# sid2364/dna-sequences-pg-extension

Hardware: AMD Instinct MI355X
Metric: k-mers/sec for k=31 count over 3 Gbase synthetic; % of HBM-read roofline (higher is better)
Workload: dtype u64; 1 GPU; config 4: k=31 count over 3000000000 synthetic bases (splitmix64 seed 0xd2a0003), unordered groups (super-k-mer partitioning), single GPU; n_bases=3000000000, k=31, distinct=2999999968

## Files before the change

dna-sequences-pg-extension_amd/__init__.py:

```python
from .binding import (
    DEBUG_FORCE_SUPERKMER,
    DEBUG_GUARD_POOL,
    DEBUG_HEAVY_EXPAND,
    DEBUG_NO_SLAB0,
    DEBUG_NO_SPEC1,
    DEBUG_POISON_POOL,
    DEBUG_RANK_SMALL,
    DEBUG_SLAB0,
    DEBUG_SLAB0_OVERFLOW,
    DEBUG_SAMPLE1,
    DEBUG_SPEC1_OVERFLOW,
    Accumulator,
    Context,
    Dna,
    DnaGpuError,
    Filter,
    Hist,
    KmerIndex,
    Records,
    SPECTRUM_MAX_BINS,
    TOP_MAX,
    MULTI_AUTO,
    MULTI_COPY,
    MULTI_RCCL,
    Multi,
    ORDER_COUNT_ASC,
    ORDER_COUNT_DESC,
    Ranking,
    abi_version,
    device_count,
    kmer_count,
    lib,
# ... 4 lines not shown
```

dna-sequences-pg-extension_amd/binding.py:

```python
import ctypes as C
import os

import numpy as np

_HERE = os.path.dirname(os.path.abspath(__file__))
_LIB = None

OK = 0
ERR_INVALID_K = 1
ERR_QKMER_LEN_MISMATCH = 2
ERR_PREFIX_TOO_LONG = 3
ERR_QKMER_INVALID = 4
ERR_BAD_ARG = 5
ERR_TOO_LARGE = 6
ERR_NO_DEVICE = 7
ERR_OOM = 8
ERR_HIP = 9
ERR_DNA_EMPTY = 11
ERR_DNA_INVALID_CHAR = 12
DEBUG_POISON_POOL = 1
DEBUG_FORCE_SUPERKMER = 2
DEBUG_HEAVY_EXPAND = 4
DEBUG_GUARD_POOL = 8
DEBUG_NO_SPEC1 = 16
DEBUG_SPEC1_OVERFLOW = 32
DEBUG_SLAB0 = 64
DEBUG_NO_SLAB0 = 128
DEBUG_SLAB0_OVERFLOW = 256
DEBUG_SAMPLE1 = 512
DEBUG_RANK_SMALL = 1024
SPECTRUM_MAX_BINS = 1 << 20
TOP_MAX = 1 << 20
ORDER_COUNT_DESC = 0
ORDER_COUNT_ASC = 1
U64_MAX = 2 ** 64 - 1


def _env_debug():
    f = 0
    if os.environ.get("DNAGPU_TEST_POISON", "0") not in ("", "0"):
        f |= DEBUG_POISON_POOL
    if os.environ.get("DNAGPU_TEST_GUARD", "0") not in ("", "0"):
        f |= DEBUG_GUARD_POOL
    return f

FILTER_EQUALS = 1
FILTER_STARTS_WITH = 2
FILTER_CONTAINS = 3

MAX_PHASES = 48

u64p = C.POINTER(C.c_uint64)

# ... 973 lines not shown
```

dna-sequences-pg-extension_amd/csrc/kernels.hpp:

```cpp
#pragma once
#include <hip/hip_runtime.h>
#include <stdint.h>

#include "kmer_device.hpp"

namespace dnagpu {

hipError_t launch_synth(u64 *words, u64 w_begin, u64 w_end, u64 n_bases, u64 seed, u64 motif_len, hipStream_t s);
hipError_t launch_extract(const u64 *words, u64 n_words, u64 first, u64 count, int k, u64 *out_keys,
                          hipStream_t s);

constexpr int FILTER_MAX_GROUPS = 8192;
struct FilterSource {
    const u64 *words;
    u64 n_words;
    const u32 *marks;
    u64 n_mark_words;
    const u64 *seq_starts;
    u64 n_seqs;
};
void filter_bits_geometry(u64 count, u32 *n_groups, u32 *tiles_per_group);
hipError_t launch_filter_bits_count(const FilterSource &src, u64 first, u64 count, const FilterBits &fb, u32 *group_counts,
                                    hipStream_t s);
hipError_t launch_filter_bits_write(const FilterSource &src, u64 first, u64 count, const FilterBits &fb,
// ... 181 lines not shown
    const u32 *beg;
    u32 R;
    u32 C;
    int k;
    int test;
    FilterDev fd;
};
u32 index_scan_tiles(u64 C);
hipError_t launch_index_sweep_count(const IndexScanArgs &a, u32 *tile_counts, hipStream_t s);
hipError_t launch_index_sweep_write(const IndexScanArgs &a, const u32 *tile_offsets, u64 *out_rows, u64 *out_keys, u64 cap,
                                    hipStream_t s);
hipError_t launch_index_lookup(const u64 *r, u64 n, int k, const u64 *keys, u64 m, u64 *out_first, u64 *out_count, hipStream_t s);
hipError_t launch_index_read(const u64 *r, const u32 *row, int k, u64 first, u64 count, u64 *out_rows, u64 *out_keys, hipStream_t s);

int sk_min_k();
int sk_minimizer_len(int k);
int sk_tile_rows();
int sk_max_c0();
hipError_t launch_sk_level0(bool scatter, const Chunk *chunks, u32 n_chunks, const u64 *words, u64 n_words, u64 first, int k,
                            u32 c0n, u32 b1bits, u32 r0bits, u32 *hist, const u32 *tot, void *recs, hipStream_t s,
                            u32 *aux = nullptr, const u32 *marks = nullptr, u64 n_mark_words = 0);
hipError_t launch_sk_sample_chunks(Chunk *chunks, u32 n_chunks, u32 stride, u32 len, u32 n, hipStream_t s);
int sk_slab_words();
u32 sk_slab_cap(u32 est, u64 chunk_rows, u64 sampled);
hipError_t launch_sk_slab_init(const u32 *est, u32 r0bits, u32 chunk_rows, u32 sampled, u32 n_chunks, u32 *slab, Node *nodes,
                               hipStream_t s);
hipError_t launch_sk_hist1(const Node *nodes, const Chunk *chunks, u32 n_chunks, const void *recs, u32 *hist, u32 *kcount,
                           hipStream_t s, bool by_d2 = false);
hipError_t launch_sk_scatter1(const Node *nodes, const Chunk *chunks, u32 n_chunks, const void *src, void *dst, const u32 *hist,
                              const u32 *tot, hipStream_t s, bool by_d2 = false, u32 *gcur = nullptr);
u64 sk_spec_span(u32 len, int bits);
hipError_t launch_sk_spec_regions(const Node *nodes, u32 n_nodes, u32 *spec, u32 *out, u32 *gcur, hipStream_t s,
                                  const u32 *rstart = nullptr);
hipError_t launch_sk_scatter1_spec(const Node *nodes, const Chunk *chunks, u32 n_chunks, const void *src, void *dst, u32 *gcur,
                                   const u32 *spec, u32 *kcount, u32 *over, hipStream_t s, const u32 *rstart = nullptr,
                                   const u32 *rcap = nullptr);
hipError_t launch_sk_spec_nodes(const Node *nodes, u32 n_nodes, const u32 *spec, const u32 *gcur, Node *next, u32 *over,
                                hipStream_t s, const u32 *rstart = nullptr, const u32 *rcap = nullptr);
u32 sk_sample1_len();
u32 sk_sample1_every();
hipError_t launch_sk_sampled_regions(const Node *nodes, const Chunk *samples, u32 n_samples, const void *recs, u32 n_mid, u32 *est,
                                     u32 *rcap, u32 *rstart, u32 *scan_tmp, u32 *total, hipStream_t s);
hipError_t launch_sk_heavy_finals(const Node *kids, u32 n, const u32 *kcount, Node *out, hipStream_t s);
int sk_flat_slice();
hipError_t launch_sk_take_heavy(Node *mids, const u32 *idx, u32 n_heavy, const u32 *kcount, Node *out, hipStream_t s);
hipError_t launch_sk_slice_count(const Node *buckets, u32 nb, u32 *n_slices, hipStream_t s);
hipError_t launch_sk_slice_fill(const Node *buckets, u32 nb, const u32 *slice_first, u32 *slice_rec0, u32 *slice_nrec, hipStream_t s);
hipError_t launch_sk_slice_kmers(const void *recs, const u32 *slice_rec0, const u32 *slice_nrec, u32 n_slices, u32 *slice_km,
                                 hipStream_t s);
// ... 34 lines not shown
```

dna-sequences-pg-extension_amd/csrc/sk_host.hip:

```cpp
#include "host_common.hpp"

using namespace dnagpu;


constexpr u64 SK_LEAF_MEAN = 2500;
constexpr u64 SK_MID_LIMIT = (u64)1 << 27;
#ifndef SK_MID_RECORDS_LOG2
#define SK_MID_RECORDS_LOG2 16
#endif
constexpr u32 SK_MID_RECORDS = 1u << SK_MID_RECORDS_LOG2;
constexpr u64 SK_BIG_LIMIT = 0xFFFFFFFFull;
constexpr int SK_B1_MAX = 9;
constexpr u64 SK_SLAB_MIN_ROWS = (u64)1 << 29;

template <typename T>
static int alloc1(PoolScope &ps, size_t n, T **out, size_t per = 1)
{
    return ps.alloc(std::max<size_t>(n, 1) * per, out);
}

static u32 sk_chunk_len(u64 x, u64 target = 4096, u64 tile = 8192)
{
    const u64 len = std::max<u64>(4 * tile, (x + target - 1) / target);
    return (u32)((len + tile - 1) / tile * tile);
// ... 39 lines not shown
    RC_TRY(alloc1(ps, hc.n_chunks, &lv->chunks));
    RC_TRY(alloc1(ps, hc.n_chunks, &lv->hist, ROW_STRIDE));
    RC_TRY(alloc1(ps, hc.n_chunks, &lv->tot, ROW_STRIDE));
    RC_TRY(alloc1(ps, hc.n_next, &lv->next));
    HIP_TRY(launch_fill_chunks(cur, n_nodes, chunk_len, outc, nch, cur, lv->chunks, st));
    return DNAGPU_OK;
}

struct SkHeavy {
    Node *nodes = nullptr;
    u32 n = 0;
    bool counted = true;
    void *recs = nullptr;
    u64 total = 0;
};

struct SkParts {
    SkGeom g;
    int k = 0;
    u64 n_expected = 0;
    void *rec0 = nullptr;
    u64 rec0_cap = 0;
    u64 n_recs = 0;
    Node *coarse = nullptr;
    u32 n_coarse = 0;
    std::vector<u32> lens;
    void *recs = nullptr;
    Node *fin = nullptr;
    u32 n_fin = 0;
    SkHeavy heavy;
    u64 n_kmers = 0;
};

SkGeom dnagpu::sk_geometry(const dnagpu_ctx *ctx, u64 n, int k)
{
    SkGeom g;
    const u64 leaf_mean = std::min<u64>(SK_LEAF_MEAN, 225 * (u64)(k - sk_minimizer_len(k) + 2));
    const u64 n_final = std::max<u64>(n / leaf_mean, 16);
    const u64 n_mid = (n_final + 15) / 16;
    g.b1 = 1;
    while (g.b1 < SK_B1_MAX && ((u64)1 << g.b1) < n_mid)
        g.b1++;
    g.c0n = (u32)std::min<u64>((n_mid + ((u64)1 << g.b1) - 1) >> g.b1, (u64)sk_max_c0());
    g.r0bits = 1;
    while ((1u << g.r0bits) < g.c0n)
        g.r0bits++;
// ... 77 lines not shown
    RC_TRY(pool_alloc(ctx, (size_t)cap * 16, &rec0));
    ps.ptrs.push_back(rec0);
    prof_mark(ctx, "sk_scatter0");
    HIP_TRY(launch_sk_level0(true, l0.chunks, l0.n_chunks, dna->words, dna->n_words, rows.first, k, c0n, (u32)b1, (u32)r0bits,
                             l0.hist, l0.tot, rec0, st, nullptr, rows.marks, rows.n_mark_words));
    p.rec0 = rec0;
    p.rec0_cap = cap;
    p.coarse = l0.next;
    p.n_coarse = l0.n_next;
    p.n_recs = n_recs;
    return DNAGPU_OK;
}

static int sk_level0_slab(dnagpu_ctx *ctx, PoolScope &ps, SkParts &p, const SkRows &rows, bool *ok)
{
    hipStream_t st = ctx->stream;
    const dnagpu_dna *dna = rows.dna;
    const SkGeom &g = p.g;
    const int k = p.k;
    const u64 first = rows.first, n = rows.n;
    *ok = false;
    const u32 r0n = 1u << g.r0bits;
    const u64 tile = (u64)sk_tile_rows();
    Node *cur = nullptr;
    u32 chunk_rows = 0;
    SkLevel l0;
    RC_TRY(sk_level0_begin(ctx, ps, n, g.r0bits, 1024, &cur, &chunk_rows, &l0));
    if (l0.n_chunks == 0)
        return DNAGPU_OK;
    const u64 samp_len = 4 * tile, samp_stride = 64 * samp_len;
    const u32 n_samp = (u32)((n + samp_stride - 1) / samp_stride);
    u64 sampled = 0;
    for (u32 i = 0; i < n_samp; i++)
        sampled += std::min<u64>(samp_len, n - (u64)i * samp_stride);
    Chunk *samp = nullptr;
    u32 *est = nullptr, *slab = nullptr;
    Node *nodes = nullptr;
    RC_TRY(ps.alloc((size_t)n_samp, &samp));
    RC_TRY(ps.alloc((size_t)sk_max_c0(), &est));
    RC_TRY(ps.alloc((size_t)sk_slab_words(), &slab));
    RC_TRY(ps.alloc((size_t)r0n, &nodes));
    prof_mark(ctx, "sk_sample0");
    HIP_TRY(hipMemsetAsync(est, 0, (size_t)sk_max_c0() * sizeof(u32), st));
    HIP_TRY(launch_sk_sample_chunks(samp, n_samp, (u32)samp_stride, (u32)samp_len, (u32)n, st));
    HIP_TRY(launch_sk_level0(false, samp, n_samp, dna->words, dna->n_words, first, k, g.c0n, (u32)g.b1, (u32)g.r0bits, nullptr, nullptr,
                             nullptr, st, est, rows.marks, rows.n_mark_words));
    HIP_TRY(launch_sk_slab_init(est, (u32)g.r0bits, chunk_rows, (u32)sampled, l0.n_chunks, slab, nodes, st));
    std::vector<u32> h_est(r0n);
    RC_TRY(read_back(ctx, h_est.data(), est, (size_t)r0n * sizeof(u32)));
    u64 tot = 0, span = 0, span1 = 0;
    p.lens.assign(r0n, 0);
    for (u32 d = 0; d < r0n; d++) {
        tot += h_est[d];
        const u64 len = (u64)sk_slab_cap(h_est[d], chunk_rows, sampled) * l0.n_chunks;
        span += len;
        if (len > 0xFFFFFFFFull)
            return DNAGPU_OK;
        p.lens[d] = (u32)len;
        span1 += sk_spec_span((u32)len, g.b1);
    }
    if (tot == 0 || !sk_even(h_est.data(), r0n, 1.05) || span > 0xFFFFFFFFull)
        return DNAGPU_OK;
    const u64 cap = std::max<u64>(span, span1 <= 0xFFFFFFFFull ? span1 : 0);
    void *rec0 = nullptr;
    RC_TRY(pool_alloc(ctx, (size_t)std::max<u64>(cap, 1) * 16, &rec0));
    prof_mark(ctx, "sk_scatter0");
    const hipError_t e = launch_sk_level0(true, l0.chunks, l0.n_chunks, dna->words, dna->n_words, first, k, g.c0n, (u32)g.b1,
                                          (u32)g.r0bits, nullptr, nullptr, rec0, st, slab, rows.marks, rows.n_mark_words);
    u32 status[2] = {1, 0};
    int rc = e == hipSuccess ? read_back(ctx, status, slab + 18 * (size_t)sk_max_c0(), sizeof status) : DNAGPU_ERR_HIP;
    if (rc != DNAGPU_OK || status[0] || status[1] != (u32)span || (ctx->debug_flags & DNAGPU_DEBUG_SLAB0_OVERFLOW)) {
        pool_free(ctx, rec0);
        if (e != hipSuccess)
            set_err("sk_scatter0 (slabs): %s", hipGetErrorString(e));
        return rc;
    }
    ps.ptrs.push_back(rec0);
    p.rec0 = rec0;
    p.rec0_cap = cap;
    p.coarse = nodes;
    p.n_coarse = r0n;
    p.n_recs = span;
    *ok = true;
    return DNAGPU_OK;
}


struct SkL1 {
    SkLevel lv;
    u32 chunk_recs = 0;
    u32 *kcount = nullptr;
    u32 *d_lens = nullptr;
    u32 *gcur = nullptr;
    std::vector<u32> kc, rcn;
    u64 span = 0;
    u32 *rstart = nullptr, *rcapv = nullptr;
    void *rec1 = nullptr;
    bool rec1_kept = false;
};

enum class SkL1Route {
    Exact,
    Speculative,
    SpeculativeSampled,
};
// ... 76 lines not shown
    u32 total = 0;
    RC_TRY(read_back(ctx, &total, tot1, sizeof total));
    u64 chk = 0;
    for (u32 i = 0; i < n_coarse; i++)
        chk += host_lens[i];
    if ((u64)total >= chk && (u64)total <= p.rec0_cap) {
        l1.span = total;
        *route = SkL1Route::SpeculativeSampled;
    }
    return DNAGPU_OK;
}

static int sk_l1_speculative(dnagpu_ctx *ctx, PoolScope &ps, const SkParts &p, SkL1 &l1, SkL1Route route, bool *moved)
{
    hipStream_t st = ctx->stream;
    const bool sampled = route == SkL1Route::SpeculativeSampled;
    const u32 n_mid = l1.lv.n_next;
    u32 *const rstart = sampled ? l1.rstart : nullptr, *const rcapv = sampled ? l1.rcapv : nullptr;
    u32 *sp = nullptr;
    RC_TRY(ps.alloc((size_t)2 * p.n_coarse, &sp));
    u32 *status = l1.d_lens + n_mid;
    prof_mark(ctx, "sk_spec1");
    HIP_TRY(launch_sk_spec_regions(p.coarse, p.n_coarse, sp, status, l1.gcur, st, rstart));
    RC_TRY(pool_alloc(ctx, (size_t)std::max<u64>(std::max(p.n_recs, l1.span), 1) * 16, &l1.rec1));
    ps.ptrs.push_back(l1.rec1);
    prof_mark(ctx, "sk_scatter1");
    HIP_TRY(launch_sk_scatter1_spec(p.coarse, l1.lv.chunks, l1.lv.n_chunks, p.rec0, l1.rec1, l1.gcur, sp, l1.kcount, status + 2, st,
                                    rstart, rcapv));
    HIP_TRY(launch_sk_spec_nodes(p.coarse, p.n_coarse, sp, l1.gcur, l1.lv.next, status + 2, st, rstart, rcapv));
    HIP_TRY(launch_sk_node_lens(l1.lv.next, n_mid, l1.d_lens, st));
    RC_TRY(sk_l1_lens_to_host(ctx, l1, 3));
    const u32 *stw = l1.rcn.data() + n_mid;
    *moved = !((!sampled && stw[0] != (u32)l1.span) || (!sampled && stw[1]) || stw[2] ||
               (ctx->debug_flags & DNAGPU_DEBUG_SPEC1_OVERFLOW));
    if (!*moved)
        HIP_TRY(hipMemsetAsync(l1.kcount, 0, (size_t)std::max<u32>(n_mid, 1) * sizeof(u32), st));
    return DNAGPU_OK;
}

static int sk_l1_histogram(dnagpu_ctx *ctx, const SkParts &p, SkL1 &l1)
{
    hipStream_t st = ctx->stream;
    const SkLevel &lv = l1.lv;
    prof_mark(ctx, "sk_hist1");
    HIP_TRY(launch_sk_hist1(p.coarse, lv.chunks, lv.n_chunks, p.rec0, lv.hist, l1.kcount, st));
    prof_mark(ctx, "sk_prefix1");
    HIP_TRY(launch_level_prefix(p.coarse, lv.chunks, lv.n_chunks, p.n_coarse, l1.chunk_recs, lv.hist, lv.tot, st, p.n_coarse));
// ... 19 lines not shown
        set_err("super-k-mer partition lost rows: %llu of %llu", (unsigned long long)run, (unsigned long long)p.n_expected);
        return DNAGPU_ERR_INTERNAL;
    }
    if (run > 0xFFFFFFFFull)
        return DNAGPU_ERR_TOO_LARGE;
    p.n_kmers = run;
    if (!any_heavy)
        return DNAGPU_OK;
    for (u32 i = 0; i < n_mid; i++)
        if (is_heavy(i)) {
            heavy_idx->push_back(i);
            p.heavy.total += kc[i];
        }
    if (((debug_flags & DNAGPU_DEBUG_HEAVY_EXPAND) && p.heavy.total * 2 > run) || heavy_idx->size() > 32768)
        return DNAGPU_SK_SKEWED;
    return DNAGPU_OK;
}

static int sk_l1_scatter(dnagpu_ctx *ctx, PoolScope &ps, const SkParts &p, SkL1 &l1)
{
    hipStream_t st = ctx->stream;
    const SkLevel &lv = l1.lv;
    if (!l1.rec1) {
        RC_TRY(pool_alloc(ctx, (size_t)std::max<u64>(p.n_recs, 1) * 16, &l1.rec1));
        ps.ptrs.push_back(l1.rec1);
    }
    prof_mark(ctx, "sk_scatter1");
    HIP_TRY(hipMemcpyAsync(l1.gcur, lv.tot, (size_t)std::max<u32>(lv.n_chunks, 1) * ROW_STRIDE * sizeof(u32), hipMemcpyDeviceToDevice,
                           st));
    HIP_TRY(launch_sk_scatter1(p.coarse, lv.chunks, lv.n_chunks, p.rec0, l1.rec1, lv.hist, lv.tot, st, false, l1.gcur));
    return DNAGPU_OK;
}

struct SkSplit {
    SkLevel lv = {};
    u32 *kcount = nullptr;
};

static int sk_heavy_take(dnagpu_ctx *ctx, PoolScope &ps, SkParts &p, SkL1 &l1, const std::vector<u32> &heavy_idx, SkSplit *split)
{
    hipStream_t st = ctx->stream;
    const u32 nh = (u32)heavy_idx.size();
    u32 *d_idx = nullptr;
    Node *hnodes = nullptr;
    RC_TRY(ps.alloc((size_t)nh, &d_idx));
    RC_TRY(ps.alloc((size_t)nh, &hnodes));
    HIP_TRY(hipMemcpyAsync(d_idx, heavy_idx.data(), (size_t)nh * sizeof(u32), hipMemcpyHostToDevice, st));
// ... 507 lines not shown
```

dna-sequences-pg-extension_amd/csrc/superkmer_kernels.hip:

```cpp
#include <algorithm>
#include <cstdlib>
#include <type_traits>

#include "kernels.hpp"

namespace dnagpu {

constexpr int SK_NT = 256;
constexpr int SKW_ROWS = 63 * 32;
constexpr int SK_TILE_ROWS = (SK_NT / 64) * SKW_ROWS;
constexpr int SK_MAX_C0 = 256;
constexpr int SKW_LIST = 768;
__host__ __device__ constexpr u32 sk_plain_max(int w) { return (u32)(2 * SKW_ROWS * 17 / (10 * (w + 1))) < (u32)SKW_LIST ? (u32)(2 * SKW_ROWS * 17 / (10 * (w + 1))) : (u32)SKW_LIST; }

int sk_tile_rows() { return SK_TILE_ROWS; }
int sk_max_c0() { return SK_MAX_C0; }
int sk_count_cap() { return 4096; }

typedef unsigned long long ull2_t __attribute__((ext_vector_type(2)));

constexpr int SK_REC_MULTI_BIT = 58;
constexpr int SK_POS_SHIFT = 39;
constexpr u32 SK_POS_MASK = 31u;
constexpr u32 SK_GPOS_MASK = 63u;

__device__ __forceinline__ u32 sk_mix_raw(u32 t, u32 hi_bits )
{
    return __umul24(t, 0x9E3779u) + __umul24(__builtin_amdgcn_ubfe(t, 24u, hi_bits), 0x85EBCBu);
}
__device__ __forceinline__ u32 sk_mix(u32 v) { return sk_mix_raw(v, 8u); }

struct SkDigits {
    u32 d0, d1, d2;
};
__device__ __forceinline__ u32 sk_digit_word(u32 hmin) { return __umul24(hmin >> 7, 0x9E3779u); }
__device__ __forceinline__ u32 sk_digit0(u32 g, u32 c0) { return __umul24(g >> 16, c0) >> 16; }
__device__ __forceinline__ u32 sk_fine_word(u32 v) { return v * 0x9E3779B1u; }
__device__ __forceinline__ SkDigits sk_digits(u32 hmin, u32 v, u32 c0, u32 b1mask)
{
// ... 345 lines not shown
                    atomicAdd(&h[sk_digit0(sk_digit_word(fm.hm[0]), c0n)], ((u32)SKW_ROWS + lmax - 1u) / lmax);
            } else {
                sk_hist0_general<W, BATCH>(fm, words, n_words, first + ch.off + t0, lmax, mmask, c0n, h);
            }
        }
    }
    __syncthreads();
    if (accum) {
        for (u32 d = threadIdx.x; d < r0n; d += SK_NT)
            if (h[d])
                atomicAdd(&accum[d], h[d]);
        return;
    }
    u32 *row = hist + (u64)blockIdx.x * ROW_STRIDE;
    for (u32 d = threadIdx.x; d < r0n; d += SK_NT)
        row[d] = h[d];
}

struct SkBuild {
    u64 *wl;
    const u64 *wsh;
    u32 *gpos;
    const u32 *gend;
    ull2_t *recs;
    u32 fo, c0n, b1mask, mmask;
    int k, dbg;
};

template <bool BATCH>
__device__ __forceinline__ bool sk_build(const SkBuild &b, u32 wrun, int mode)
{
    const bool exact = mode != 0;
    const int dbg = b.dbg;
    (void)dbg;
    bool dropped = false;
    if (SK_DBG(2))
        return false;
    for (u32 e = threadIdx.x & 63u; e < wrun; e += 64) {
        const u64 en = b.wl[e];
        const u32 key = (u32)(en >> 32);
        if (BATCH && (exact ? key < 64u : key == ~0u))
            continue;
        const u32 end_row = (u32)en & 0xFFFFu;
        u32 v = key, hmin = key;
        if (exact) {
            const u32 xq = (end_row & ~31u) + (key & SK_GPOS_MASK) + b.fo;
// ... 9 lines not shown
        const u32 len = end_row - start + 1u;
        const u32 q = start + b.fo;
        const u32 wi = q >> 5, sh = (q & 15u) * 2u;
        const u64 a0 = b.wsh[wi], a1 = b.wsh[wi + 1], a2 = b.wsh[wi + 2];
        const bool odd = (q & 16u) != 0;
        const u32 e0 = odd ? (u32)(a0 >> 32) : (u32)a0, e1 = odd ? (u32)a1 : (u32)(a0 >> 32),
                  e2 = odd ? (u32)(a1 >> 32) : (u32)a1, e3 = odd ? (u32)a2 : (u32)(a1 >> 32),
                  e4 = odd ? (u32)(a2 >> 32) : (u32)a2;
        u64 lo = ((u64)__builtin_amdgcn_alignbit(e2, e1, sh) << 32) | __builtin_amdgcn_alignbit(e1, e0, sh);
        u64 hi = ((u64)__builtin_amdgcn_alignbit(e4, e3, sh) << 32) | __builtin_amdgcn_alignbit(e3, e2, sh);
        const u32 nb = len + (u32)b.k - 1;
        if (nb < 32) {
            lo &= ((u64)1 << (2 * nb)) - 1;
            hi = 0;
        } else {
            hi &= ((u64)1 << (2 * (nb - 32))) - 1;
        }
        const u32 mpos = (end_row & ~31u) + (key & SK_GPOS_MASK) - start;
        const u32 tag = exact ? (mpos & SK_POS_MASK) << (SK_POS_SHIFT - 32) : 1u << (SK_REC_MULTI_BIT - 32);
        hi |= ((u64)(len - 1) << 44) | ((u64)dg.d1 << 49) | ((u64)dg.d2 << 59) | ((u64)tag << 32);
        ull2_t r;
        r.x = lo;
        r.y = hi;
        if (gslot >= b.gend[dg.d0])
            dropped = true;
        else if (!SK_DBG(1))
            b.recs[gslot] = r;
        else if (r.x == 0x1234567 && r.y == 0x89)
            b.recs[0] = r;
    }
    return dropped;
}

template <int W, bool BATCH, bool BYV>
__device__ __forceinline__ bool sk_scatter0_walk(SkFront<W> &f, const SkBuild &bx, const u64 *__restrict__ words, u64 n_words,
                                                 u64 tile_pos, u32 lmax)
{
    const u64 below = ((u64)1 << (threadIdx.x & 63)) - 1;
    u64 *wl = bx.wl;
    bool dropped = false;
    SkKeys<W, BATCH, BYV> key(f, words, n_words, tile_pos, bx.mmask);
    sk_front_open<W>(f, key, lmax);
    for (int n_pass = BYV ? 1 : 4, pass = 0; pass < n_pass; pass++) {
        const int jlo = pass * (32 / n_pass), jhi = jlo + 32 / n_pass;
        u32 wrun = 0;
        key.forget();
        sk_records_all<W>(f, key, lmax, [&](int j, bool end_any, u32 end_row, u32 len, u32, u32 kj) {
            const bool end = end_any && j >= jlo && j < jhi;
            const u64 b = __ballot(end);
// ... 45 lines not shown
        for (u32 d = tid; d < r0n; d += SK_NT) {
            const u32 cap = slab[d];
            const u32 base = cap ? atomicAdd(&slab[SK_MAX_C0 + 16 * d], cap) : 0u;
            gpos[d] = base;
            gbeg[d] = base;
            gend[d] = base + cap;
        }
    } else {
        const u32 *hrow = hist + (u64)blockIdx.x * ROW_STRIDE;
        const u32 *trow = tot;
        for (u32 d = tid; d < r0n; d += SK_NT) {
            gpos[d] = trow[d] + hrow[d];
            gend[d] = ~0u;
        }
    }
    __syncthreads();
    u64 *wsh = wsh_all[wave], *wl = list_all[wave];
    bool dropped = false;
    SkBuild bx;
    bx.wl = wl;
    bx.wsh = wsh;
    bx.gpos = gpos;
    bx.gend = gend;
    bx.recs = recs;
    bx.fo = 0;
    bx.c0n = c0n;
    bx.b1mask = b1mask;
    bx.mmask = mmask;
    bx.k = k;
    bx.dbg = dbg;
    for (u32 t0 = (u32)wave * SKW_ROWS; t0 < ch.len; t0 += SK_TILE_ROWS) {
        const u32 n_rows = ch.len - t0 < (u32)SKW_ROWS ? ch.len - t0 : (u32)SKW_ROWS;
        const u64 tile_pos = first + ch.off + t0;
        const u32 fo = (u32)(tile_pos & 31);
        SkFront<W> f;
        sk_front<W, BATCH>(f, words, n_words, tile_pos, n_rows, lmax, mmask, wsh, marks, n_mark_words);
        bx.fo = fo;
        auto build = [&](u32 wrun, int mode) {
            if (sk_build<BATCH>(bx, wrun, mode))
                dropped = true;
        };
        if (f.plain) {
            const u32 nf = lane == 62 ? ~f.hm[31] : f.next_first;
            u32 cnt = 0;
#pragma unroll
            for (int j = 0; j < 32; j++)
// ... 19 lines not shown
            }
        }
        {
            SkFront<W> fm = f;
            const SkBuild bm = bx;
            const u32 uv = fm.plain ? sk_uniform_value<W, BATCH>(fm, words, n_words, tile_pos, mmask) : ~0u;
            if (uv != ~0u) {
                const u32 n_rec = ((u32)SKW_ROWS + lmax - 1u) / lmax;
                for (u32 e = (u32)lane; e < n_rec; e += 64) {
                    const u32 s0 = e * lmax, e1 = (s0 + lmax < (u32)SKW_ROWS ? s0 + lmax : (u32)SKW_ROWS) - 1u;
                    wl[e] = ((u64)uv << 32) | (u64)((s0 << 16) | e1);
                }
                sk_wave_fence();
                if (sk_build<BATCH>(bm, n_rec, 0))
                    dropped = true;
                sk_wave_fence();
            } else if (sk_scatter0_general<W, BATCH>(fm, bm, words, n_words, tile_pos, lmax)) {
                dropped = true;
            }
        }
    }
    if (slab) {
        if (dropped)
            slab[18 * SK_MAX_C0] = 1u;
        __syncthreads();
        ull2_t null_rec;
        null_rec.x = 0;
        null_rec.y = (unsigned long long)1 << 63;
        for (u32 d = (u32)wave; d < r0n; d += SK_NT / 64) {
            const u32 e = gend[d], u = gpos[d] < e ? gpos[d] : e;
            for (u32 i = u + (u32)lane; i < e; i += 64)
                __builtin_nontemporal_store(null_rec, &recs[i]);
            if (lane == 0 && u > gbeg[d])
                atomicAdd(&slab[17 * SK_MAX_C0 + d], u - gbeg[d]);
        }
    }
}

__global__ __launch_bounds__(256) void sk_sample_chunks_kernel(Chunk *__restrict__ chunks, u32 n_chunks, u32 stride, u32 len, u32 n)
{
    const u32 i = blockIdx.x * blockDim.x + threadIdx.x;
    if (i >= n_chunks)
        return;
    const u64 off = (u64)i * stride;
    Chunk c;
    c.node = 0;
    c.off = (u32)off;
    c.len = off >= (u64)n ? 0u : (u32)((u64)len < (u64)n - off ? (u64)len : (u64)n - off);
    c.pad = 0;
    chunks[i] = c;
}

__host__ __device__ inline u32 sk_isqrt(u64 v)
{
    u64 r = 0, bit = (u64)1 << 62;
    while (bit > v)
        bit >>= 2;
    while (bit) {
        if (v >= r + bit) {
            v -= r + bit;
            r = (r >> 1) + bit;
        } else {
            r >>= 1;
        }
        bit >>= 2;
    }
    return (u32)r;
}
__host__ __device__ inline u32 sk_slab_cap_of(u32 est, u64 chunk_rows, u64 sampled)
{
    if (est == 0)
        return 0;
    const u64 e = ((u64)est * chunk_rows) / sampled + 1;
    return (u32)((e + e / 32 + 6 * (u64)sk_isqrt(e) + 24 + 7) & ~(u64)7);
}
u32 sk_slab_cap(u32 est, u64 chunk_rows, u64 sampled) { return sk_slab_cap_of(est, chunk_rows, sampled); }

__global__ __launch_bounds__(SK_MAX_C0) void sk_slab_init_kernel(const u32 *__restrict__ est, u32 r0n, u32 chunk_rows, u32 sampled,
                                                                u32 n_chunks, u32 child_meta, u32 *__restrict__ slab,
                                                                Node *__restrict__ nodes)
{
    __shared__ u64 sc[SK_MAX_C0];
    const u32 d = threadIdx.x;
    const u32 cap = d < r0n ? sk_slab_cap_of(est[d], chunk_rows, sampled) : 0u;
    sc[d] = (u64)cap * n_chunks;
    __syncthreads();
    if (d == 0) {
        u64 run = 0;
        for (u32 i = 0; i < (u32)SK_MAX_C0; i++) {
            const u64 c = sc[i];
            sc[i] = run;
            run += c;
        }
        slab[18 * SK_MAX_C0] = 0;
        slab[18 * SK_MAX_C0 + 1] = (u32)(run < 0xFFFFFFFFull ? run : 0xFFFFFFFFull);
    }
    __syncthreads();
    if (d < r0n) {
        const u32 start = (u32)(sc[d] < 0xFFFFFFFFull ? sc[d] : 0xFFFFFFFFull);
        slab[d] = cap;
        slab[SK_MAX_C0 + 16 * d] = start;
        slab[17 * SK_MAX_C0 + d] = 0;
        Node o;
        o.start = start;
        o.len = cap * n_chunks;
        o.meta = child_meta;
        o.split = 0;
        o.prefix = 0;
        o.child_base = 0;
        o.chunk_base = 0;
        nodes[d] = o;
    }
}

constexpr int SK1_NT = 1024;
__global__ __launch_bounds__(SK1_NT) void sk_hist1_kernel(const Node *__restrict__ nodes, const Chunk *__restrict__ chunks,
                                                          u32 n_chunks, const ull2_t *__restrict__ recs,
                                                          u32 *__restrict__ hist, u32 *__restrict__ kcount, int shift)
{
    __shared__ u32 h[ROW_STRIDE];
    __shared__ u32 kc[ROW_STRIDE];
    if (blockIdx.x >= n_chunks)
        return;
    const Chunk ch = chunks[blockIdx.x];
    const Node nd = nodes[ch.node];
    const u32 R = 1u << nd.split;
    for (u32 d = threadIdx.x; d < R; d += SK1_NT) {
        h[d] = 0;
        kc[d] = 0;
    }
    __syncthreads();
    const u64 *hi = reinterpret_cast<const u64 *>(recs + (u64)nd.start + ch.off) + 1;
    u32 i = threadIdx.x;
    for (; i + 3u * SK1_NT < ch.len; i += 4u * SK1_NT) {
        u64 m[4];
// ... 1918 lines not shown
    const u32 b1mask = (1u << b1bits) - 1, r0n = 1u << r0bits;
    if (r0n > (u32)SK_MAX_C0)
        return hipErrorInvalidValue;
#define SK_CASE(W_) case W_: \
        if (marks) launch_front<W_, true>(scatter, n_chunks, s, chunks, words, n_words, first, k, lmax, mmask, c0n, b1mask, r0n, hist, tot, recs, aux, marks, n_mark_words); \
        else launch_front<W_, false>(scatter, n_chunks, s, chunks, words, n_words, first, k, lmax, mmask, c0n, b1mask, r0n, hist, tot, recs, aux, nullptr, 0); \
        break;
    switch (w) {
        SK_CASE(9) SK_CASE(10) SK_CASE(11) SK_CASE(12) SK_CASE(13) SK_CASE(14) SK_CASE(15) SK_CASE(16) SK_CASE(17) SK_CASE(18)
    default: return hipErrorInvalidValue;
    }
#undef SK_CASE
    return hipGetLastError();
}

hipError_t launch_sk_sample_chunks(Chunk *chunks, u32 n_chunks, u32 stride, u32 len, u32 n, hipStream_t s)
{
    if (n_chunks == 0)
        return hipSuccess;
    hipLaunchKernelGGL(sk_sample_chunks_kernel, dim3((n_chunks + 255) / 256), dim3(256), 0, s, chunks, n_chunks, stride, len, n);
    return hipGetLastError();
}

int sk_slab_words() { return 18 * SK_MAX_C0 + 4; }

hipError_t launch_sk_slab_init(const u32 *est, u32 r0bits, u32 chunk_rows, u32 sampled, u32 n_chunks, u32 *slab, Node *nodes,
                               hipStream_t s)
{
    hipLaunchKernelGGL(sk_slab_init_kernel, dim3(1), dim3(SK_MAX_C0), 0, s, est, 1u << r0bits, chunk_rows, sampled, n_chunks,
                       (u32)(32 - r0bits), slab, nodes);
    return hipGetLastError();
}

hipError_t launch_sk_hist1(const Node *nodes, const Chunk *chunks, u32 n_chunks, const void *recs, u32 *hist, u32 *kcount,
                           hipStream_t s, bool by_d2)
{
    if (n_chunks == 0)
        return hipSuccess;
    hipLaunchKernelGGL(sk_hist1_kernel, dim3(n_chunks), dim3(SK1_NT), 0, s, nodes, chunks, n_chunks,
                       reinterpret_cast<const ull2_t *>(recs), hist, kcount, by_d2 ? 59 : 49);
    return hipGetLastError();
}

hipError_t launch_sk_scatter1(const Node *nodes, const Chunk *chunks, u32 n_chunks, const void *src, void *dst, const u32 *hist,
                              const u32 *tot, hipStream_t s, bool by_d2, u32 *gcur)
{
    if (n_chunks == 0)
        return hipSuccess;
    hipLaunchKernelGGL(sk_scatter1_kernel<false>, dim3(n_chunks), dim3(SK1_NT), 0, s, nodes, chunks, n_chunks,
                       reinterpret_cast<const ull2_t *>(src), reinterpret_cast<ull2_t *>(dst), hist, tot, by_d2 ? 59 : 49, gcur,
                       nullptr, nullptr, nullptr, nullptr, nullptr);
    return hipGetLastError();
}
// ... 75 lines not shown
```

include/dnagpu.h:

```cpp
#ifndef DNAGPU_H
#define DNAGPU_H

#include <stdint.h>
#include <stddef.h>

#ifdef __cplusplus
extern "C" {
#endif

#define DNAGPU_ABI_VERSION 2

#define DNAGPU_OK                       0
#define DNAGPU_ERR_INVALID_K            1
#define DNAGPU_ERR_QKMER_LEN_MISMATCH   2
#define DNAGPU_ERR_PREFIX_TOO_LONG      3
#define DNAGPU_ERR_QKMER_INVALID        4
#define DNAGPU_ERR_BAD_ARG              5
#define DNAGPU_ERR_TOO_LARGE            6
#define DNAGPU_ERR_NO_DEVICE            7
#define DNAGPU_ERR_OOM                  8
#define DNAGPU_ERR_HIP                  9
#define DNAGPU_ERR_INTERNAL             10
#define DNAGPU_ERR_DNA_EMPTY            11
#define DNAGPU_ERR_DNA_INVALID_CHAR     12
// ... 202 lines not shown
int dnagpu_kmer_index_build(dnagpu_ctx *ctx, const uint64_t *keys, uint64_t n, int k, int on_device, dnagpu_kmer_index **out);
uint64_t dnagpu_kmer_index_rows(const dnagpu_kmer_index *idx);
uint64_t dnagpu_kmer_index_distinct(const dnagpu_kmer_index *idx);
int dnagpu_kmer_index_k(const dnagpu_kmer_index *idx);
int dnagpu_kmer_index_scan(dnagpu_ctx *ctx, const dnagpu_kmer_index *idx, const dnagpu_filter *filter, uint64_t *out_rows,
                           uint64_t *out_keys, uint64_t cap, uint64_t *n_out, uint64_t *visited, int out_on_device);
int dnagpu_kmer_index_lookup(dnagpu_ctx *ctx, const dnagpu_kmer_index *idx, const uint64_t *keys, uint64_t m,
                             uint64_t *out_first, uint64_t *out_count, int on_device);
int dnagpu_kmer_index_read(dnagpu_ctx *ctx, const dnagpu_kmer_index *idx, uint64_t first, uint64_t count, uint64_t *out_rows,
                           uint64_t *out_keys, int out_on_device);
void dnagpu_kmer_index_free(dnagpu_ctx *ctx, dnagpu_kmer_index *idx);

#define DNAGPU_DEBUG_POISON_POOL 1u
#define DNAGPU_DEBUG_FORCE_SUPERKMER 2u
#define DNAGPU_DEBUG_HEAVY_EXPAND 4u
#define DNAGPU_DEBUG_GUARD_POOL 8u
#define DNAGPU_DEBUG_NO_SPEC1 16u
#define DNAGPU_DEBUG_SPEC1_OVERFLOW 32u
#define DNAGPU_DEBUG_SLAB0 64u
#define DNAGPU_DEBUG_NO_SLAB0 128u
#define DNAGPU_DEBUG_SLAB0_OVERFLOW 256u
#define DNAGPU_DEBUG_SAMPLE1 512u
#define DNAGPU_DEBUG_RANK_SMALL 1024u
int dnagpu_set_debug(dnagpu_ctx *ctx, unsigned flags);

#define DNAGPU_MAX_PHASES 48
typedef struct dnagpu_phase_times {
    int         n;
    const char *names[DNAGPU_MAX_PHASES];
    float       ms[DNAGPU_MAX_PHASES];
} dnagpu_phase_times;
int dnagpu_last_phase_times(dnagpu_ctx *ctx, dnagpu_phase_times *out);
int dnagpu_multi_last_phase_times(dnagpu_multi *m, int rank, dnagpu_phase_times *out);
int dnagpu_set_profiling(dnagpu_ctx *ctx, int enabled);

#ifdef __cplusplus
}
#endif
#endif
```

Measured before the change: 164.7 billion k-mers/s.

## Add per-bucket overflow areas to level-0 slab scatter and shrink slab padding

New measurement: 167.1 billion k-mers/s (median of 3 runs). About the same (+1.5%).

```diff
diff --git a/dna-sequences-pg-extension_amd/__init__.py b/dna-sequences-pg-extension_amd/__init__.py
--- a/dna-sequences-pg-extension_amd/__init__.py
+++ b/dna-sequences-pg-extension_amd/__init__.py
@@ -7,7 +7,9 @@
     DEBUG_POISON_POOL,
     DEBUG_RANK_SMALL,
     DEBUG_SLAB0,
+    DEBUG_SLAB0_NO_AREA,
     DEBUG_SLAB0_OVERFLOW,
+    DEBUG_SLAB0_TIGHT,
     DEBUG_SAMPLE1,
     DEBUG_SPEC1_OVERFLOW,
     Accumulator,
diff --git a/dna-sequences-pg-extension_amd/binding.py b/dna-sequences-pg-extension_amd/binding.py
--- a/dna-sequences-pg-extension_amd/binding.py
+++ b/dna-sequences-pg-extension_amd/binding.py
@@ -29,6 +29,8 @@
 DEBUG_SLAB0_OVERFLOW = 256
 DEBUG_SAMPLE1 = 512
 DEBUG_RANK_SMALL = 1024
+DEBUG_SLAB0_TIGHT = 2048
+DEBUG_SLAB0_NO_AREA = 4096
 SPECTRUM_MAX_BINS = 1 << 20
 TOP_MAX = 1 << 20
 ORDER_COUNT_DESC = 0
diff --git a/dna-sequences-pg-extension_amd/csrc/kernels.hpp b/dna-sequences-pg-extension_amd/csrc/kernels.hpp
--- a/dna-sequences-pg-extension_amd/csrc/kernels.hpp
+++ b/dna-sequences-pg-extension_amd/csrc/kernels.hpp
@@ -227,9 +227,12 @@
                             u32 *aux = nullptr, const u32 *marks = nullptr, u64 n_mark_words = 0);
 hipError_t launch_sk_sample_chunks(Chunk *chunks, u32 n_chunks, u32 stride, u32 len, u32 n, hipStream_t s);
 int sk_slab_words();
-u32 sk_slab_cap(u32 est, u64 chunk_rows, u64 sampled);
-hipError_t launch_sk_slab_init(const u32 *est, u32 r0bits, u32 chunk_rows, u32 sampled, u32 n_chunks, u32 *slab, Node *nodes,
-                               hipStream_t s);
+constexpr u32 SK_SLAB_TIGHT = 1, SK_SLAB_NO_AREA = 2;
+u32 sk_slab_cap(u32 est, u64 chunk_rows, u64 sampled, u32 mode);
+u64 sk_slab_area(u32 est, u64 chunk_rows, u64 sampled, u32 n_chunks, u32 mode);
+hipError_t launch_sk_slab_init(const u32 *est, u32 r0bits, u32 chunk_rows, u32 sampled, u32 n_chunks, u32 mode, u32 *slab,
+                               Node *nodes, hipStream_t s);
+hipError_t launch_sk_slab_close(u32 r0bits, u32 *slab, Node *nodes, hipStream_t s);
 hipError_t launch_sk_hist1(const Node *nodes, const Chunk *chunks, u32 n_chunks, const void *recs, u32 *hist, u32 *kcount,
                            hipStream_t s, bool by_d2 = false);
 hipError_t launch_sk_scatter1(const Node *nodes, const Chunk *chunks, u32 n_chunks, const void *src, void *dst, const u32 *hist,
diff --git a/dna-sequences-pg-extension_amd/csrc/sk_host.hip b/dna-sequences-pg-extension_amd/csrc/sk_host.hip
--- a/dna-sequences-pg-extension_amd/csrc/sk_host.hip
+++ b/dna-sequences-pg-extension_amd/csrc/sk_host.hip
@@ -85,6 +85,7 @@
     void *rec0 = nullptr;
     u64 rec0_cap = 0;
     u64 n_recs = 0;
+    u64 rec0_span = 0;
     Node *coarse = nullptr;
     u32 n_coarse = 0;
     std::vector<u32> lens;
@@ -208,6 +209,8 @@
     *ok = false;
     const u32 r0n = 1u << g.r0bits;
     const u64 tile = (u64)sk_tile_rows();
+    const u32 mode = ((ctx->debug_flags & DNAGPU_DEBUG_SLAB0_TIGHT) ? SK_SLAB_TIGHT : 0u) |
+                     ((ctx->debug_flags & DNAGPU_DEBUG_SLAB0_NO_AREA) ? SK_SLAB_NO_AREA : 0u);
     Node *cur = nullptr;
     u32 chunk_rows = 0;
     SkLevel l0;
@@ -231,18 +234,18 @@
     HIP_TRY(launch_sk_sample_chunks(samp, n_samp, (u32)samp_stride, (u32)samp_len, (u32)n, st));
     HIP_TRY(launch_sk_level0(false, samp, n_samp, dna->words, dna->n_words, first, k, g.c0n, (u32)g.b1, (u32)g.r0bits, nullptr, nullptr,
                              nullptr, st, est, rows.marks, rows.n_mark_words));
-    HIP_TRY(launch_sk_slab_init(est, (u32)g.r0bits, chunk_rows, (u32)sampled, l0.n_chunks, slab, nodes, st));
+    HIP_TRY(launch_sk_slab_init(est, (u32)g.r0bits, chunk_rows, (u32)sampled, l0.n_chunks, mode, slab, nodes, st));
     std::vector<u32> h_est(r0n);
     RC_TRY(read_back(ctx, h_est.data(), est, (size_t)r0n * sizeof(u32)));
-    u64 tot = 0, span = 0, span1 = 0;
-    p.lens.assign(r0n, 0);
+    u64 tot = 0, span = 0, span1 = 0, slab_slots = 0;
     for (u32 d = 0; d < r0n; d++) {
         tot += h_est[d];
-        const u64 len = (u64)sk_slab_cap(h_est[d], chunk_rows, sampled) * l0.n_chunks;
+        const u64 slabs = (u64)sk_slab_cap(h_est[d], chunk_rows, sampled, mode) * l0.n_chunks;
+        const u64 len = slabs + sk_slab_area(h_est[d], chunk_rows, sampled, l0.n_chunks, mode);
+        slab_slots += slabs;
         span += len;
         if (len > 0xFFFFFFFFull)
             return DNAGPU_OK;
-        p.lens[d] = (u32)len;
         span1 += sk_spec_span((u32)len, g.b1);
     }
     if (tot == 0 || !sk_even(h_est.data(), r0n, 1.05) || span > 0xFFFFFFFFull)
@@ -251,22 +254,41 @@
     void *rec0 = nullptr;
     RC_TRY(pool_alloc(ctx, (size_t)std::max<u64>(cap, 1) * 16, &rec0));
     prof_mark(ctx, "sk_scatter0");
-    const hipError_t e = launch_sk_level0(true, l0.chunks, l0.n_chunks, dna->words, dna->n_words, first, k, g.c0n, (u32)g.b1,
-                                          (u32)g.r0bits, nullptr, nullptr, rec0, st, slab, rows.marks, rows.n_mark_words);
-    u32 status[2] = {1, 0};
-    int rc = e == hipSuccess ? read_back(ctx, status, slab + 18 * (size_t)sk_max_c0(), sizeof status) : DNAGPU_ERR_HIP;
+    hipError_t e = launch_sk_level0(true, l0.chunks, l0.n_chunks, dna->words, dna->n_words, first, k, g.c0n, (u32)g.b1,
+                                    (u32)g.r0bits, nullptr, nullptr, rec0, st, slab, rows.marks, rows.n_mark_words);
+    if (e == hipSuccess)
+        e = launch_sk_slab_close((u32)g.r0bits, slab, nodes, st);
+    std::vector<u32> status(4 + (size_t)r0n, 0);
+    status[0] = 1;
+    int rc = e == hipSuccess ? read_back(ctx, status.data(), slab + 18 * (size_t)sk_max_c0(), status.size() * sizeof(u32))
+                             : DNAGPU_ERR_HIP;
     if (rc != DNAGPU_OK || status[0] || status[1] != (u32)span || (ctx->debug_flags & DNAGPU_DEBUG_SLAB0_OVERFLOW)) {
         pool_free(ctx, rec0);
         if (e != hipSuccess)
             set_err("sk_scatter0 (slabs): %s", hipGetErrorString(e));
         return rc;
     }
+    u64 n_recs = 0;
+    p.lens.assign(status.begin() + 4, status.end());
+    for (u32 d = 0; d < r0n; d++)
+        n_recs += p.lens[d];
+#ifdef DNAGPU_STAMPS
+    fprintf(stderr, "[sk slab0] %llu slots in slabs, %llu records through the overflow areas, %llu slots allocated\n",
+            (unsigned long long)slab_slots, (unsigned long long)(n_recs - slab_slots), (unsigned long long)span);
+#endif
+    if (n_recs < slab_slots || n_recs > span) {
+        set_err("sk_scatter0 (slabs): %llu slots used, %llu in slabs, %llu allocated", (unsigned long long)n_recs,
+                (unsigned long long)slab_slots, (unsigned long long)span);
+        pool_free(ctx, rec0);
+        return DNAGPU_ERR_INTERNAL;
+    }
     ps.ptrs.push_back(rec0);
     p.rec0 = rec0;
     p.rec0_cap = cap;
+    p.rec0_span = span;
     p.coarse = nodes;
     p.n_coarse = r0n;
-    p.n_recs = span;
+    p.n_recs = n_recs;
     *ok = true;
     return DNAGPU_OK;
 }
@@ -389,7 +411,7 @@
     u32 *status = l1.d_lens + n_mid;
     prof_mark(ctx, "sk_spec1");
     HIP_TRY(launch_sk_spec_regions(p.coarse, p.n_coarse, sp, status, l1.gcur, st, rstart));
-    RC_TRY(pool_alloc(ctx, (size_t)std::max<u64>(std::max(p.n_recs, l1.span), 1) * 16, &l1.rec1));
+    RC_TRY(pool_alloc(ctx, (size_t)std::max<u64>(std::max({p.n_recs, p.rec0_span, l1.span}), 1) * 16, &l1.rec1));
     ps.ptrs.push_back(l1.rec1);
     prof_mark(ctx, "sk_scatter1");
     HIP_TRY(launch_sk_scatter1_spec(p.coarse, l1.lv.chunks, l1.lv.n_chunks, p.rec0, l1.rec1, l1.gcur, sp, l1.kcount, status + 2, st,
@@ -455,7 +477,7 @@
     hipStream_t st = ctx->stream;
     const SkLevel &lv = l1.lv;
     if (!l1.rec1) {
-        RC_TRY(pool_alloc(ctx, (size_t)std::max<u64>(p.n_recs, 1) * 16, &l1.rec1));
+        RC_TRY(pool_alloc(ctx, (size_t)std::max<u64>(std::max(p.n_recs, p.rec0_span), 1) * 16, &l1.rec1));
         ps.ptrs.push_back(l1.rec1);
     }
     prof_mark(ctx, "sk_scatter1");
diff --git a/dna-sequences-pg-extension_amd/csrc/superkmer_kernels.hip b/dna-sequences-pg-extension_amd/csrc/superkmer_kernels.hip
--- a/dna-sequences-pg-extension_amd/csrc/superkmer_kernels.hip
+++ b/dna-sequences-pg-extension_amd/csrc/superkmer_kernels.hip
@@ -15,6 +15,12 @@
 
 int sk_tile_rows() { return SK_TILE_ROWS; }
 int sk_max_c0() { return SK_MAX_C0; }
+constexpr u32 SK_SLAB_STATUS = 18 * SK_MAX_C0;
+constexpr u32 SK_SLAB_LENS = SK_SLAB_STATUS + 4;
+constexpr u32 SK_SLAB_OCUR = 20 * SK_MAX_C0;
+constexpr u32 SK_SLAB_OBEG = 36 * SK_MAX_C0;
+constexpr u32 SK_SLAB_OEND = 37 * SK_MAX_C0;
+constexpr int SK_SLAB_WORDS = 38 * SK_MAX_C0;
 int sk_count_cap() { return 4096; }
 
 typedef unsigned long long ull2_t __attribute__((ext_vector_type(2)));
@@ -406,6 +412,7 @@
     const u64 *wsh;
     u32 *gpos;
     const u32 *gend;
+    u32 *ovf;
     ull2_t *recs;
     u32 fo, c0n, b1mask, mmask;
     int k, dbg;
@@ -461,9 +468,15 @@
         ull2_t r;
         r.x = lo;
         r.y = hi;
-        if (gslot >= b.gend[dg.d0])
-            dropped = true;
-        else if (!SK_DBG(1))
+        if (gslot >= b.gend[dg.d0]) {
+            u32 *oc = b.ovf + SK_SLAB_OCUR + 16u * dg.d0;
+            const u32 beg = b.ovf[SK_SLAB_OBEG + dg.d0], room = b.ovf[SK_SLAB_OEND + dg.d0] - beg;
+            const u32 o = atomicAdd(oc, 1u);
+            if (o - beg < room)
+                b.recs[o] = r;
+            else
+                dropped = true;
+        } else if (!SK_DBG(1))
             b.recs[gslot] = r;
         else if (r.x == 0x1234567 && r.y == 0x89)
             b.recs[0] = r;
@@ -555,6 +568,7 @@
     bx.wsh = wsh;
     bx.gpos = gpos;
     bx.gend = gend;
+    bx.ovf = slab;
     bx.recs = recs;
     bx.fo = 0;
     bx.c0n = c0n;
@@ -620,7 +634,7 @@
     }
     if (slab) {
         if (dropped)
-            slab[18 * SK_MAX_C0] = 1u;
+            slab[SK_SLAB_STATUS] = 1u;
         __syncthreads();
         ull2_t null_rec;
         null_rec.x = 0;
@@ -665,23 +679,43 @@
     }
     return (u32)r;
 }
-__host__ __device__ inline u32 sk_slab_cap_of(u32 est, u64 chunk_rows, u64 sampled)
-{
-    if (est == 0)
+__host__ __device__ inline u64 sk_slab_share(u32 est, u64 chunk_rows, u64 sampled)
+{
+    return est ? ((u64)est * chunk_rows) / sampled + 1 : 0;
+}
+__host__ __device__ inline u32 sk_slab_cap_of(u32 est, u64 chunk_rows, u64 sampled, u32 mode)
+{
+    const u64 e = sk_slab_share(est, chunk_rows, sampled);
+    if (e == 0)
         return 0;
-    const u64 e = ((u64)est * chunk_rows) / sampled + 1;
-    return (u32)((e + e / 32 + 6 * (u64)sk_isqrt(e) + 24 + 7) & ~(u64)7);
-}
-u32 sk_slab_cap(u32 est, u64 chunk_rows, u64 sampled) { return sk_slab_cap_of(est, chunk_rows, sampled); }
+    if (mode & SK_SLAB_TIGHT) {
+        const u64 c = (3 * e / 4) & ~(u64)7;
+        return (u32)(c > 8 ? c : 8);
+    }
+    return (u32)((e + e / 64 + (u64)sk_isqrt(e) + 8 + 7) & ~(u64)7);
+}
+__host__ __device__ inline u64 sk_slab_area_of(u32 est, u64 chunk_rows, u64 sampled, u32 n_chunks, u32 mode)
+{
+    if (mode & SK_SLAB_NO_AREA)
+        return 0;
+    const u64 E = sk_slab_share(est, chunk_rows, sampled) * n_chunks;
+    return (E / ((mode & SK_SLAB_TIGHT) ? 2 : 32) + 6 * (u64)sk_isqrt(E) + 64 + 7) & ~(u64)7;
+}
+u32 sk_slab_cap(u32 est, u64 chunk_rows, u64 sampled, u32 mode) { return sk_slab_cap_of(est, chunk_rows, sampled, mode); }
+u64 sk_slab_area(u32 est, u64 chunk_rows, u64 sampled, u32 n_chunks, u32 mode)
+{
+    return sk_slab_area_of(est, chunk_rows, sampled, n_chunks, mode);
+}
 
 __global__ __launch_bounds__(SK_MAX_C0) void sk_slab_init_kernel(const u32 *__restrict__ est, u32 r0n, u32 chunk_rows, u32 sampled,
-                                                                u32 n_chunks, u32 child_meta, u32 *__restrict__ slab,
+                                                                u32 n_chunks, u32 mode, u32 child_meta, u32 *__restrict__ slab,
                                                                 Node *__restrict__ nodes)
 {
     __shared__ u64 sc[SK_MAX_C0];
     const u32 d = threadIdx.x;
-    const u32 cap = d < r0n ? sk_slab_cap_of(est[d], chunk_rows, sampled) : 0u;
-    sc[d] = (u64)cap * n_chunks;
+    const u32 cap = d < r0n ? sk_slab_cap_of(est[d], chunk_rows, sampled, mode) : 0u;
+    const u64 slabs = (u64)cap * n_chunks, area = d < r0n ? sk_slab_area_of(est[d], chunk_rows, sampled, n_chunks, mode) : 0;
+    sc[d] = slabs + area;
     __syncthreads();
     if (d == 0) {
         u64 run = 0;
@@ -690,18 +724,24 @@
             sc[i] = run;
             run += c;
         }
-        slab[18 * SK_MAX_C0] = 0;
-        slab[18 * SK_MAX_C0 + 1] = (u32)(run < 0xFFFFFFFFull ? run : 0xFFFFFFFFull);
+        slab[SK_SLAB_STATUS] = 0;
+        slab[SK_SLAB_STATUS + 1] = (u32)(run < 0xFFFFFFFFull ? run : 0xFFFFFFFFull);
     }
     __syncthreads();
     if (d < r0n) {
         const u32 start = (u32)(sc[d] < 0xFFFFFFFFull ? sc[d] : 0xFFFFFFFFull);
+        const u32 obeg = (u32)(sc[d] + slabs < 0xFFFFFFFFull ? sc[d] + slabs : 0xFFFFFFFFull);
+        const u32 oend = (u32)(sc[d] + slabs + area < 0xFFFFFFFFull ? sc[d] + slabs + area : 0xFFFFFFFFull);
         slab[d] = cap;
         slab[SK_MAX_C0 + 16 * d] = start;
         slab[17 * SK_MAX_C0 + d] = 0;
+        slab[SK_SLAB_LENS + d] = 0;
+        slab[SK_SLAB_OCUR + 16 * d] = obeg;
+        slab[SK_SLAB_OBEG + d] = obeg;
+        slab[SK_SLAB_OEND + d] = oend;
         Node o;
         o.start = start;
-        o.len = cap * n_chunks;
+        o.len = obeg - start;
         o.meta = child_meta;
         o.split = 0;
         o.prefix = 0;
@@ -709,6 +749,22 @@
         o.chunk_base = 0;
         nodes[d] = o;
     }
+}
+
+__global__ __launch_bounds__(SK_MAX_C0) void sk_slab_close_kernel(u32 r0n, u32 *__restrict__ slab, Node *__restrict__ nodes)
+{
+    const u32 d = threadIdx.x;
+    if (d >= r0n)
+        return;
+    const u32 beg = slab[SK_SLAB_OBEG + d], room = slab[SK_SLAB_OEND + d] - beg;
+    const u32 drawn = slab[SK_SLAB_OCUR + 16 * d] - beg;
+    const u32 used = drawn < room ? drawn : room;
+    if (drawn > room)
+        slab[SK_SLAB_STATUS] = 1u;
+    const u32 len = beg - nodes[d].start + used;
+    nodes[d].len = len;
+    slab[SK_SLAB_LENS + d] = len;
+    slab[17 * SK_MAX_C0 + d] += used;
 }
 
 constexpr int SK1_NT = 1024;
@@ -2673,13 +2729,23 @@
     return hipGetLastError();
 }
 
-int sk_slab_words() { return 18 * SK_MAX_C0 + 4; }
-
-hipError_t launch_sk_slab_init(const u32 *est, u32 r0bits, u32 chunk_rows, u32 sampled, u32 n_chunks, u32 *slab, Node *nodes,
-                               hipStream_t s)
-{
-    hipLaunchKernelGGL(sk_slab_init_kernel, dim3(1), dim3(SK_MAX_C0), 0, s, est, 1u << r0bits, chunk_rows, sampled, n_chunks,
+int sk_slab_words() { return SK_SLAB_WORDS; }
+
+hipError_t launch_sk_slab_init(const u32 *est, u32 r0bits, u32 chunk_rows, u32 sampled, u32 n_chunks, u32 mode, u32 *slab,
+                               Node *nodes, hipStream_t s)
+{
+    if (r0bits > 8)
+        return hipErrorInvalidValue;
+    hipLaunchKernelGGL(sk_slab_init_kernel, dim3(1), dim3(SK_MAX_C0), 0, s, est, 1u << r0bits, chunk_rows, sampled, n_chunks, mode,
                        (u32)(32 - r0bits), slab, nodes);
+    return hipGetLastError();
+}
+
+hipError_t launch_sk_slab_close(u32 r0bits, u32 *slab, Node *nodes, hipStream_t s)
+{
+    if (r0bits > 8)
+        return hipErrorInvalidValue;
+    hipLaunchKernelGGL(sk_slab_close_kernel, dim3(1), dim3(SK_MAX_C0), 0, s, 1u << r0bits, slab, nodes);
     return hipGetLastError();
 }
 
diff --git a/include/dnagpu.h b/include/dnagpu.h
--- a/include/dnagpu.h
+++ b/include/dnagpu.h
@@ -248,6 +248,8 @@
 #define DNAGPU_DEBUG_SLAB0_OVERFLOW 256u
 #define DNAGPU_DEBUG_SAMPLE1 512u
 #define DNAGPU_DEBUG_RANK_SMALL 1024u
+#define DNAGPU_DEBUG_SLAB0_TIGHT 2048u
+#define DNAGPU_DEBUG_SLAB0_NO_AREA 4096u
 int dnagpu_set_debug(dnagpu_ctx *ctx, unsigned flags);
 
 #define DNAGPU_MAX_PHASES 48
```
